# saghen/frizbee

Measured on AMD Instinct MI355X. Metric: haystacks scored/sec (whole node) + achieved HBM GB/s, 6-char needle vs 10M len-32 haystacks, higher is better.
Workload: dtype u8; 1 GPU; needle 'deadbe' (6 chars) vs 10,000,000 x 32-byte ASCII haystacks per GPU, max_typos=0, mix 5% full / 20% partial / 75% none, seed 12345 (BASELINE.json configs[1]); haystacks_per_gpu=10000000, haystack_len=32, max_typos=0, emulated_reference_backend=AVX-512 (prefilter 64 lanes, Smith-Waterman 64 x u8), ranks_seen=1, backend=none (single process), filter_survivors=499537

## Files before the change

frizbee_amd/csrc/dp_cf.h:

```cpp
#pragma once
#include "dp_body.h"

constexpr bool cf_entry_lane(int k, int s, int P) {
    if (k < 0 || k >= P) return false;
    if (s == 1) return k == P - 1;
    const int lo = P - s > 0 ? P - s : 0, hi = P - s / 2 > 0 ? P - s / 2 : 0;
    return k >= lo && k < hi;
}

struct CfRow {
    u32 orv, cmpv, cv;
    bool ci;
};
struct NeedleLongRows : NeedleLongDev {
    const u16* cf;
};
template <typename ND>
__device__ __forceinline__ CfRow cf_row_consts(const ND& nd, u32 r) {
    u32 c, f;
    if constexpr (ND::kLong) {
        const u32 cf = nd.cf[r];
        c = cf & 0xFF, f = cf >> 8;
    } else {
        c = (((const u32*)nd.c)[r >> 2] >> (8 * (r & 3))) & 0xFF, f = (((const u32*)nd.f)[r >> 2] >> (8 * (r & 3))) & 0xFF;
    }
    CfRow k;
    k.ci = c != f;
    k.orv = k.ci ? 0x00200020u : 0u;
    k.cmpv = splat16(k.ci ? (c | 0x20) : c);
    k.cv = splat16(c);
    return k;
}

template <bool UPPER>
__device__ __forceinline__ void cf_match(const CfRow& k, u32 hw, u32 bonus, u32 casev, u32& mm, u32& mb) {
    const u32 ONE = 0x00010001u;
    mm = p_subs(ONE, (hw | k.orv) ^ k.cmpv);
    mb = p_mul(mm, bonus);
    if (UPPER) {
        const u32 ex = k.ci ? p_subs(ONE, hw ^ k.cv) : mm;
        mb = p_add(mb, p_mul(ex, casev));
    }
}

template <int SWL, int REAL>
__device__ __forceinline__ void cf_scan(u32 (&b)[REAL], const u32 (&g)[REAL], u32 e, u32 lim, u32& acc0, u32& acc1) {
    constexpr int NW = SWL / 2, P = 2 * REAL;
    constexpr bool PAD = REAL < NW;
    {
        u32 cc[REAL], nb[REAL];
#pragma unroll
        for (int d = 0; d < REAL; d++) cc[d] = p_subs(b[d], g[d]);
        if (PAD && e < lim) acc1 = p_max(acc1, p_subs(cc[REAL - 1], 0xFFFFu | (((u32)P * e) << 16)));
#pragma unroll
        for (int d = 0; d < REAL; d++) nb[d] = p_max(b[d], __builtin_amdgcn_alignbit(cc[d], d ? cc[d - 1] : 0u, 16));
#pragma unroll
        for (int d = 0; d < REAL; d++) b[d] = nb[d];
    }
#pragma unroll
    for (int s = 2; s <= SWL / 2; s *= 2) {
        const int off = s / 2;
        if (PAD && (u32)s * e < lim) {
#pragma unroll
            for (int d = 0; d < REAL; d++) {
                const bool in0 = cf_entry_lane(2 * d, s, P), in1 = cf_entry_lane(2 * d + 1, s, P);
                if (in0 || in1) {
                    const u32 k0 = in0 ? (u32)(2 * d + s) * e : 0xFFFFu, k1 = in1 ? (u32)(2 * d + 1 + s) * e : 0xFFFFu;
                    const u32 v = p_subs(p_subs(b[d], g[d]), k0 | (k1 << 16));
                    if (d & 1) acc1 = p_max(acc1, v);
                    else acc0 = p_max(acc0, v);
                }
            }
        }
        if (off < REAL) {
            u32 nb[REAL];
#pragma unroll
            for (int d = 0; d < REAL; d++) nb[d] = d >= off ? p_max(b[d], p_subs(b[d - off], g[d - off])) : b[d];
#pragma unroll
            for (int d = 0; d < REAL; d++) b[d] = nb[d];
        }
    }
}

struct CfNoRowHook {
    __device__ __forceinline__ void operator()() const {}
};

template <int SWL, bool UPPER, int REAL, typename RowHook = CfNoRowHook>
__device__ __forceinline__ u32 cf_rows(const NeedleDev& nd, const u32 (&hw)[REAL], const u32 (&bonus)[REAL], const RowHook& hook = RowHook()) {
    constexpr int NW = SWL / 2;
    constexpr int P = 2 * REAL;
    constexpr bool PAD = REAL < NW;
    static_assert(REAL >= 1 && REAL <= NW, "REAL");
    static_assert(!PAD || 4 * P <= 3 * SWL, "padding entries must land inside the chunk");
    const u32 rows = (u32)nd.rows;
    const u32 e = nd.gex, x = nd.mismatch, o = nd.gopm;
    const u32 ev = splat16(e), gopmv = splat16(o), casev = splat16(nd.matching_case);
    const u32 xv = splat16(x), xqv = splat16(x - 2 * e);
    if (rows == 1) {
        const CfRow k = cf_row_consts(nd, 0);
        u32 mx = 0;
#pragma unroll
        for (int d = 0; d < REAL; d++) {
            u32 mm, mb;
            cf_match<UPPER>(k, hw[d], bonus[d], casev, mm, mb);
            mx = p_max(mx, p_subs(mb, xv));
        }
        return max(mx & 0xFFFF, mx >> 16);
    }
    u32 T[REAL], g[REAL];
    u32 acc0 = 0, acc1 = 0;
    {
        const CfRow k = cf_row_consts(nd, 0);
        u32 bias = e + (e << 17);
#pragma unroll
        for (int d = 0; d < REAL; d++, bias = fzb_sadd(bias, 2 * ev)) {
            u32 mm, mb;
            cf_match<UPPER>(k, hw[d], bonus[d], casev, mm, mb);
            T[d] = p_max(p_subs(p_add(mb, bias), xv), bias);
            g[d] = p_mul(mm, gopmv);
        }
        cf_scan<SWL, REAL>(T, g, e, (rows - 2) * o, acc0, acc1);
    }
    const u32 edc = 0xFFFFu | (((u32)(P - 2) * e + x) << 16);
    for (u32 r = 1; r + 1 < rows; r++) {
        if (r == rows / 2) hook();
        const CfRow k = cf_row_consts(nd, r);
        const u32 rb = (r + 1) * ev;
        const u32 z = ((r - 1) * e) << 16;
        if (PAD) acc0 = p_max(acc0, p_subs(T[REAL - 1], edc));
        u32 b[REAL], gn[REAL];
        u32 bias = (e << 16) + rb;
#pragma unroll
        for (int d = 0; d < REAL; d++, bias = fzb_sadd(bias, 2 * ev)) {
            const u32 sh = __builtin_amdgcn_alignbit(T[d], d ? T[d - 1] : z, 16);
            u32 mm, mb;
            cf_match<UPPER>(k, hw[d], bonus[d], casev, mm, mb);
            const u32 D = p_subs(p_add(sh, mb), xqv);
            const u32 U = p_subs(T[d], g[d]);
            b[d] = p_max3_s(D, U, bias);
            gn[d] = p_mul(mm, gopmv);
        }
        cf_scan<SWL, REAL>(b, gn, e, (rows - 2 - r) * o, acc0, acc1);
#pragma unroll
        for (int d = 0; d < REAL; d++) T[d] = b[d], g[d] = gn[d];
    }
    u32 mx;
    {
        const u32 r = rows - 1;
        const CfRow k = cf_row_consts(nd, r);
        const u32 rb = (r + 1) * ev;
        const u32 z = ((r - 1) * e) << 16;
        if (PAD) acc0 = p_max(acc0, p_subs(T[REAL - 1], edc));
        mx = p_subs(p_max(acc0, acc1), rb);
        u32 bias = (e << 16) + rb;
#pragma unroll
        for (int d = 0; d < REAL; d++, bias = fzb_sadd(bias, 2 * ev)) {
            const u32 sh = __builtin_amdgcn_alignbit(T[d], d ? T[d - 1] : z, 16);
            u32 mm, mb;
            cf_match<UPPER>(k, hw[d], bonus[d], casev, mm, mb);
            const u32 D = p_subs(p_add(sh, mb), xqv);
            const u32 U = p_subs(T[d], g[d]);
            mx = p_max(mx, p_subs(p_max(D, U), bias));
        }
    }
    return max(mx & 0xFFFF, mx >> 16);
}

template <int SWL, bool UPPER, int REAL>
__device__ __forceinline__ void cf_setup_bits(const NeedleDev& nd, bool include_prefix, const u8* cls, const u32 (&hb)[SWL / 4], u32 (&hw)[REAL], u32 (&bonus)[REAL]) {
    const u32 ONE = 0x00010001u;
    const u32 Mv = splat16(nd.match_plus_mismatch), casev = splat16(nd.matching_case), capv = splat16(nd.capitalization), delimv = splat16(nd.delimiter);
    u32 clsw_prev = 0;
#pragma unroll
    for (int d = 0; d < REAL; d++) {
        const u32 w = hb[d / 2];
        const u32 b0 = (d & 1) ? (w >> 16) & 0xFF : w & 0xFF;
        const u32 b1 = (d & 1) ? w >> 24 : (w >> 8) & 0xFF;
        hw[d] = b0 | (b1 << 16);
        const u32 clsw = (u32)cls[b0] | ((u32)cls[b1] << 16);
        const u32 sh = __builtin_amdgcn_alignbit(clsw, clsw_prev, 16);
        const u32 cap01 = (clsw >> 1) & sh & ONE;
        const u32 dl01 = (sh >> 2) & ~(clsw >> 2) & ONE;
        u32 bn = p_add(p_add(p_mul(dl01, delimv), p_mul(cap01, capv)), Mv);
        if (d == 0 && include_prefix) bn = p_add(bn, (u32)nd.prefix);
        bonus[d] = UPPER ? bn : p_add(bn, p_mul(~(clsw >> 1) & ONE, casev));
        clsw_prev = clsw;
    }
}

struct CfTables {
    u8 cls2[256];
    u16 bon[16];
};
template <bool UPPER, typename ND = NeedleDev>
__device__ __forceinline__ void cf_build_tables(const ND& nd, CfTables& t) {
    for (int b = threadIdx.x; b < 256; b += blockDim.x) {
        const bool lower = b >= 'a' && b <= 'z', upper = b >= 'A' && b <= 'Z', digit = b >= '0' && b <= '9';
        const bool delim = !(lower || upper || digit || b > 127);
        t.cls2[b] = (u8)(2 * (lower ? 1 : upper ? 2 : delim ? 3 : 0));
    }
    if (threadIdx.x < 16) {
        const u32 cp = threadIdx.x >> 2, cc = threadIdx.x & 3;
        u32 v = nd.match_plus_mismatch;
        if (cp == 3 && cc != 3) v += nd.delimiter;
        if (cc == 2 && cp == 1) v += nd.capitalization;
        if (!UPPER && cc != 2) v += nd.matching_case;
        t.bon[threadIdx.x] = (u16)v;
    }
}
template <int SWL, int REAL>
__device__ __forceinline__ void cf_setup_table(const NeedleDev& nd, bool include_prefix, const CfTables& t, const u32 (&hb)[SWL / 4], u32 (&hw)[REAL], u32 (&bonus)[REAL]) {
    u32 cprev = 0;
#pragma unroll
    for (int d = 0; d < REAL; d++) {
        hw[d] = __builtin_amdgcn_perm(0u, hb[d / 2], (d & 1) ? 0x0c030c02u : 0x0c010c00u);
        const u32 c0 = t.cls2[hw[d] & 0xFF], c1 = t.cls2[hw[d] >> 16];
// ... 72 lines not shown
```

frizbee_amd/csrc/kernels_dp.hip:

```cpp
#include "dp_cfm.h"
#include "dp_quad.h"
#include "compact1.h"
#include "seg_list.h"
#include <cstdlib>
#include <type_traits>

template <int SWL, int MODE, bool UPPER>
__global__ __launch_bounds__(128, 2) void k2b_dp(const u8* __restrict__ bytes, const EndsAny ends, u64 first, u32 index_offset,
                                              const u32* __restrict__ items, const u32* __restrict__ win, const u32* __restrict__ n_items_ptr,
                                              const NeedleDev nd, int wmode, int pad_ok, fzb_match_rec* __restrict__ out, u32 capacity, u32* __restrict__ dev_count,
                                              u32* __restrict__ overflow, u32 qcap, u32* __restrict__ counters) {
    __shared__ u8 cls[256];
    build_cls_table(cls);
    __syncthreads();
    const u32 M = __builtin_amdgcn_readfirstlane(*n_items_ptr);
    if (dev_count && blockIdx.x == 0 && threadIdx.x == 0) { dev_count[0] = M < capacity ? M : capacity; dev_count[1] = M; }
    const u64 stride = (u64)gridDim.x * blockDim.x;
    const u64 j0 = (u64)blockIdx.x * blockDim.x + threadIdx.x;
    auto load_item = [&](u64 j, u32& li, u32& ws, u32& we) {
        li = 0; ws = 0; we = 0;
        if (j < M) {
            li = items ? items[j] : (u32)j;
            if (wmode == 0) { const uint2 w = *(const uint2*)(win + 2 * j); ws = w.x; we = w.y; }
        }
// ... 42 lines not shown
            const u32 m = we - sp;
            const bool wide = m > (u32)SWL, greedy = m > FZB_MAX_HAYSTACK_LEN;
            const u32 slot_multi = wave_alloc(&counters[3], wide && !greedy);
            const u32 slot_greedy = wave_alloc(&counters[4], greedy);
            if (wide) {
                u32* qe = greedy ? overflow + 4 * (size_t)(qcap - 1 - slot_greedy) : overflow + 4 * (size_t)slot_multi;
                qe[0] = (u32)j;
                qe[1] = ws;
                qe[2] = we;
                qe[3] = li;
                break;
            }
            u32 score = 0;
            u32 hb[SWL / 4];
#pragma unroll
            for (int k = 0; k < SWL / 4; k++) hb[k] = 0;
            if (m > 0) {
                if (inreg) load_window_regs<SWL / 4>(q0_c, q1_c, sp, m, hb);
                else load_window_mem<SWL / 4>(hay + sp, m, hb);
                const bool half = pad_ok && SWL >= 16 && __all((int)(m <= (u32)SWL / 2));
                if (half) score = dp_single_chunk<SWL, MODE == 1, UPPER, (SWL >= 16 ? SWL / 4 : SWL / 2)>(nd, m, sp == 0, cls, hb);
                else score = dp_single_chunk<SWL, MODE == 1, UPPER>(nd, m, sp == 0, cls, hb);
            }
            const bool exact = exact_match<SWL / 4>(nd, include_exact, m, hb);
            if (exact) score = (score + nd.exact_bonus) & 0xFFFF;
            fzb_match_rec rec;
            rec.index = index_offset + li;
            rec.score = (u16)score;
            rec.exact = exact ? 1 : 0;
            rec.valid = 0;
            out[j] = rec;
        } while (0);
        li_c = li_n; ws_c = ws_n; we_c = we_n; s_c = s_n; L_c = L_n; q0_c = q0_n; q1_c = q1_n;
        li_n = li_m; ws_n = ws_m; we_n = we_m; s_n = s_m; L_n = L_m;
        li_m = li_f; ws_m = ws_f; we_m = we_f;
    }
}

#ifdef FZB_DP_TIMING
__device__ unsigned long long fzb_dp_timing[6 * 8192];
extern "C" int fzb_debug_dp_timing(unsigned long long* host_out) { return (int)hipMemcpyFromSymbol(host_out, HIP_SYMBOL(fzb_dp_timing), sizeof(fzb_dp_timing)); }
#define FZB_TIMING_BEGIN const unsigned long long t_rt0 = wall_clock64(), t_ck0 = clock64();
#define FZB_TIMING_END                                                                                  \
    if ((threadIdx.x & 63) == 0) {                                                                      \
        const u32 w = (blockIdx.x * blockDim.x + threadIdx.x) >> 6;                                     \
        if (w < 8192) { fzb_dp_timing[6 * w] = t_rt0; fzb_dp_timing[6 * w + 1] = wall_clock64(); fzb_dp_timing[6 * w + 2] = t_ck0; fzb_dp_timing[6 * w + 3] = clock64(); \
                        fzb_dp_timing[6 * w + 4] = __builtin_amdgcn_s_getreg(4 | (31 << 11)); fzb_dp_timing[6 * w + 5] = __builtin_amdgcn_s_getreg(20 | (31 << 11)); }  \
    }
#else
#define FZB_TIMING_BEGIN
#define FZB_TIMING_END
#endif
struct SegNone {};
template <int SWL, bool UPPER, bool SEG = false>
__global__ __launch_bounds__(128, 4) void k2b_dp_short(const u8* __restrict__ bytes, const EndsAny ends, u64 first, u32 index_offset,
                                                    const u32* __restrict__ items, const u32* __restrict__ win, const u32* __restrict__ n_items_ptr,
                                                    const NeedleDev nd, int wmode, fzb_match_rec* __restrict__ out, u32 capacity, u32* __restrict__ dev_count,
                                                    RejectOut rej, u32* __restrict__ kept_out, u32 ulen, std::conditional_t<SEG, SegList, SegNone> seg) {
    FZB_TIMING_BEGIN
    __shared__ CfTables tab;
    __shared__ u8 fl[256];
    __shared__ u32 seg_pre[SEG ? FZB_SEG_MAX : 1u];
    __shared__ u32 seg_wsum[2];
    u32 sc[16];
    if constexpr (SEG) {
        const uint4* c4 = (const uint4*)seg.counts;
#pragma unroll
        for (int k = 0; k < 4; k++) {
            const u32 i0 = 16u * threadIdx.x + 4u * k;
            const uint4 v = i0 < seg.nseg ? c4[4 * threadIdx.x + k] : make_uint4(0, 0, 0, 0);
            sc[4 * k] = v.x;
            sc[4 * k + 1] = i0 + 1 < seg.nseg ? v.y : 0u;
            sc[4 * k + 2] = i0 + 2 < seg.nseg ? v.z : 0u;
            sc[4 * k + 3] = i0 + 3 < seg.nseg ? v.w : 0u;
        }
    }
    cf_build_tables<UPPER>(nd, tab);
    if (wmode == 3) cf_build_typo_table(nd, fl);
    u32 seg_incl = 0, seg_tot = 0;
    if constexpr (SEG) {
#pragma unroll
        for (int k = 0; k < 16; k++) seg_tot += sc[k];
        seg_incl = seg_tot;
        for (int off = 1; off < 64; off <<= 1) {
            const u32 v = __shfl_up(seg_incl, off);
            if ((threadIdx.x & 63) >= (u32)off) seg_incl += v;
        }
        if ((threadIdx.x & 63) == 63) seg_wsum[threadIdx.x >> 6] = seg_incl;
    }
    __syncthreads();
    u32 M_;
    if constexpr (SEG) {
        u32 run = (threadIdx.x >= 64 ? seg_wsum[0] : 0u) + seg_incl - seg_tot;
#pragma unroll
        for (int k = 0; k < 16; k++) {
            seg_pre[16 * threadIdx.x + k] = run;
            run += sc[k];
        }
        M_ = seg_wsum[0] + seg_wsum[1];
        __syncthreads();
        if (blockIdx.x == 0 && threadIdx.x == 0) *seg.total_out = M_;
    } else {
        M_ = *n_items_ptr;
    }
    const u32 M = __builtin_amdgcn_readfirstlane(M_);
    const u32 nrej = wmode == 3 ? __builtin_amdgcn_readfirstlane(*rej.count) : 0u;
    if (blockIdx.x == 0 && threadIdx.x == 0) {
        const u32 kept = M - nrej;
        if (dev_count) { dev_count[0] = kept < capacity ? kept : capacity; dev_count[1] = kept; }
        if (kept_out) *kept_out = kept;
    }
    const u64 stride = (u64)gridDim.x * blockDim.x;
    const u64 j0 = (u64)blockIdx.x * blockDim.x + threadIdx.x;
    auto load_item = [&](u64 j, u32& li, u32& ws, u32& we) {
        li = 0; ws = 0; we = 0;
        if (j < M) {
            if constexpr (SEG) {
                const u32 sg = seg_find(seg_pre, FZB_SEG_MAX, FZB_SEG_MAX / 2, (u32)j);
                li = seg.list[(size_t)sg * seg.stride + ((u32)j - seg_pre[sg])];
            } else {
                li = items ? items[j] : (u32)j;
            }
            if (wmode == 0) { const uint2 w = *(const uint2*)(win + 2 * j); ws = w.x; we = w.y; }
        }
    };
    auto load_span = [&](u64 j, u32 li, u64& s, u32& L) {
        s = 0; L = 0;
        if (j < M) haystack_span_u(ends, ulen, first + li, s, L);
    };
    auto load_vecs = [&](u64 s, u32 L, uint4& q0, uint4& q1) {
        q0 = make_uint4(0, 0, 0, 0);
        q1 = make_uint4(0, 0, 0, 0);
        const uint4* vp = (const uint4*)(bytes + s);
        if (L > 0) q0 = vp[0];
        if (SWL > 32 && L > 16) q1 = vp[1];
    };
    u32 li_c, ws_c, we_c, L_c, li_n, ws_n, we_n, L_n, li_m, ws_m, we_m;
    u64 s_c, s_n;
    uint4 q0_c, q1_c;
    load_item(j0, li_c, ws_c, we_c);
    load_item(j0 + stride, li_n, ws_n, we_n);
    load_item(j0 + 2 * stride, li_m, ws_m, we_m);
    load_span(j0, li_c, s_c, L_c);
    load_span(j0 + stride, li_n, s_n, L_n);
    load_vecs(s_c, L_c, q0_c, q1_c);
    const u32 jw = __builtin_amdgcn_readfirstlane((u32)j0);
    const u32 n_iter = __builtin_amdgcn_readfirstlane(jw < M ? (u32)(((u64)M - jw + stride - 1) / stride) : 1u);
    struct MidItem {
        FzbProgressPrio* p;
        __device__ __forceinline__ void operator()() const { p->k2 += 1; p->apply(); }
    };
    FzbProgressPrio prio{0u, 2 * n_iter};
    for (u64 j = j0; j < M; j += stride) {
        prio.apply();
        uint4 q0_n, q1_n;
        load_vecs(s_n, L_n, q0_n, q1_n);
        u64 s_m;
        u32 L_m;
        load_span(j + 2 * stride, li_m, s_m, L_m);
        u32 li_f, ws_f, we_f;
        load_item(j + 3 * stride, li_f, ws_f, we_f);
        u64 jo = j;
        bool live = true;
        if (nrej) {
            const u32 li = li_c, tile = li / FZB_TILE;
            const u64 word = rej.bits[li >> 6];
            live = !((word >> (li & 63)) & 1);
            u32 before = rej.rej_prefix[tile] + (u32)__popcll(word & ((1ull << (li & 63)) - 1));
            for (u32 wq = tile * (FZB_TILE / 64); wq < (li >> 6); wq++) before += (u32)__popcll(rej.bits[wq]);
            jo = j - before;
        }
        if (live && jo < capacity) {
            const u32 L = L_c;
            u32 ws = ws_c, we = we_c;
            if (wmode == 2) { ws = 0; we = L; }
            else if (wmode == 1) cf_window_first_last_regs(nd, q0_c, q1_c, ws, we);
            else if (wmode == 3) cf_window_typos_regs(fl, q0_c, q1_c, L, ws, we);
            const u32 sp = ws ? ws - 1 : 0;
            const bool include_exact = sp == 0 && we == L;
            const u32 m = we - sp;
            u32 score = 0;
            u32 hb[SWL / 4];
#pragma unroll
            for (int k = 0; k < SWL / 4; k++) hb[k] = 0;
            if (m > 0) {
                load_window_regs<SWL / 4>(q0_c, q1_c, sp, m, hb);
                score = dp_single_chunk_cf_tab<SWL, UPPER, SWL / 4, MidItem>(nd, sp == 0, tab, hb, MidItem{&prio});
            }
            const bool exact = exact_match<SWL / 4>(nd, include_exact, m, hb);
            if (exact) score = (score + nd.exact_bonus) & 0xFFFF;
            fzb_match_rec rec;
            rec.index = index_offset + li_c;
            rec.score = (u16)score;
            rec.exact = exact ? 1 : 0;
            rec.valid = 0;
            out[jo] = rec;
        }
        li_c = li_n; ws_c = ws_n; we_c = we_n; s_c = s_n; L_c = L_n; q0_c = q0_n; q1_c = q1_n;
        li_n = li_m; ws_n = ws_m; we_n = we_m; s_n = s_m; L_n = L_m;
        li_m = li_f; ws_m = ws_f; we_m = we_f;
        prio.k2 = (prio.k2 | 1u) + 1;
    }
    FZB_TIMING_END
}

template <int PER>
__device__ __forceinline__ void classify_tile(u32 j0, u32 j_end, u32* s_cnt, u32* s_base, const u8* __restrict__ bytes, const EndsAny& ends, u64 first, const u32* __restrict__ items,
                                              const u32* __restrict__ win_in, const NeedleDev& nd, int wmode, u32 swl, uint4* __restrict__ meta, u32* __restrict__ lists, u32 list_stride,
                                              u32* __restrict__ overflow, u32 qcap, u32* __restrict__ counters, u32 capacity, u32 split_multi) {
    if (threadIdx.x < 9) s_cnt[threadIdx.x] = 0;
    __syncthreads();
    u32 cls[PER], rank[PER], li[PER], ws[PER], we[PER];
    const u8* src[PER];
#pragma unroll
    for (int p = 0; p < PER; p++) {
        const u32 j = j0 + p * 256 + threadIdx.x;
        cls[p] = 9; rank[p] = 0; li[p] = 0; ws[p] = 0; we[p] = 0; src[p] = bytes;
        if (j < j_end && j < capacity) {
            li[p] = items ? items[j] : j;
            u32 L = 0;
            u64 s;
            haystack_span(ends, first + li[p], s, L);
            src[p] = bytes + s;
            if (wmode == 0) { ws[p] = win_in[2 * j]; we[p] = win_in[2 * j + 1]; }
            else if (wmode == 2) { ws[p] = 0; we[p] = L; }
            else window_first_last(nd, src[p], L, ws[p], we[p]);
            const u32 sp = ws[p] ? ws[p] - 1 : 0;
            const u32 m = we[p] - sp;
            if (sp == 0 && we[p] == L) we[p] |= 0x80000000u;
            cls[p] = m <= swl / 2 ? 0u : m <= 3 * swl / 4 ? 1u : m <= swl ? 2u : m <= FZB_MAX_HAYSTACK_LEN ? 3u : 4u;
            if (split_multi && cls[p] == 3) cls[p] = 5 + ((m - 1) % swl) / (swl / 4);
            rank[p] = atomicAdd(&s_cnt[cls[p]], 1u);
        }
    }
    __syncthreads();
    if (threadIdx.x < 9 && s_cnt[threadIdx.x]) {
        const u32 c = threadIdx.x;
        s_base[c] = atomicAdd(c < 3 ? &counters[8 + c] : c == 3 ? &counters[3] : c == 4 ? &counters[4] : &counters[12 + (c - 5)], s_cnt[c]);
    }
    __syncthreads();
#pragma unroll
    for (int p = 0; p < PER; p++) {
        const u32 j = j0 + p * 256 + threadIdx.x;
        if (cls[p] < 3 || (cls[p] >= 5 && cls[p] < 9)) {
            const u32 l = cls[p] < 3 ? cls[p] : cls[p] - 2;
            lists[(size_t)l * list_stride + s_base[cls[p]] + rank[p]] = j;
            meta[j] = make_uint4(ws[p], we[p], (u32)(uintptr_t)src[p], (u32)((uintptr_t)src[p] >> 32));
        } else if (cls[p] < 5) {
            const u32 slot = s_base[cls[p]] + rank[p];
// ... 51 lines not shown
    const u32 stride = vgrid * blockDim.x;
    const u32 q0 = vblock * blockDim.x + threadIdx.x;
    auto load_meta = [&](u32 q, u32& j, u32& li, u32& sp, u32& m, u32& L, u64& s) {
        j = 0; li = 0; sp = 0; m = 0; L = 0; s = (u64)(uintptr_t)meta;
        if (q < M) {
            j = list[q];
            li = items ? items[j] : j;
            const uint4 w = meta[j];
            sp = w.x ? w.x - 1 : 0;
            m = (w.y & 0x7FFFFFFFu) - sp;
            L = w.y >> 31;
            s = (u64)w.z | ((u64)w.w << 32);
        }
    };
    auto load_bytes = [&](u64 s, u32 sp, u32 m, u32 (&hb)[NBR]) {
        const u8* th = (const u8*)(uintptr_t)s + sp;
#pragma unroll
        for (int k = 0; k < NBR; k++) {
            const u32 p = 4 * k;
            u32 v = 0;
            if (p < m) {
                v = load_u32_unaligned(th, p);
                const u32 rem = m - p;
                if (rem < 4) v &= (1u << (8 * rem)) - 1;
            }
            hb[k] = v;
        }
    };
    u32 j_c, li_c, sp_c, m_c, ex_c, j_n, li_n, sp_n, m_n, ex_n;
    u64 s_c, s_n;
    u32 hb_c[NBR];
    load_meta(q0, j_c, li_c, sp_c, m_c, ex_c, s_c);
    load_meta(q0 + stride, j_n, li_n, sp_n, m_n, ex_n, s_n);
    load_bytes(s_c, sp_c, m_c, hb_c);
    const u32 qw = __builtin_amdgcn_readfirstlane(q0);
    const u32 n_iter = __builtin_amdgcn_readfirstlane(qw < M ? (M - qw + stride - 1) / stride : 1u);
    struct MidItem {
        FzbProgressPrio* p;
        __device__ __forceinline__ void operator()() const { p->k2 += 1; p->apply(); }
    };
    FzbProgressPrio prio{0u, 2 * n_iter};
    for (u32 q = q0; q < M; q += stride) {
        prio.apply();
        u32 hb_n[NBR];
        load_bytes(s_n, sp_n, m_n, hb_n);
        u32 j_f, li_f, sp_f, m_f, ex_f;
        u64 s_f;
        load_meta(q + 2 * stride, j_f, li_f, sp_f, m_f, ex_f, s_f);
        {
            u32 hb[NB];
#pragma unroll
            for (int k = 0; k < NB; k++) hb[k] = k < NBR ? hb_c[k < NBR ? k : 0] : 0u;
            u32 score = 0;
            if (m_c > 0) score = dp_single_chunk_cf_tab<SWL, UPPER, REAL, MidItem>(nd, sp_c == 0, tab, hb, MidItem{&prio});
            const bool exact = exact_match<NB>(nd, ex_c != 0, m_c, hb);
            if (exact) score = (score + nd.exact_bonus) & 0xFFFF;
            fzb_match_rec rec;
            rec.index = index_offset + li_c;
            rec.score = (u16)score;
            rec.exact = exact ? 1 : 0;
            rec.valid = 0;
            out[j_c] = rec;
        }
        j_c = j_n; li_c = li_n; sp_c = sp_n; m_c = m_n; ex_c = ex_n; s_c = s_n;
#pragma unroll
        for (int k = 0; k < NBR; k++) hb_c[k] = hb_n[k];
        j_n = j_f; li_n = li_f; sp_n = sp_f; m_n = m_f; ex_n = ex_f; s_n = s_f;
        prio.k2 = (prio.k2 | 1u) + 1;
    }
}

template <int SWL, bool UPPER, int REAL>
__global__ __launch_bounds__(128, (REAL * 4 <= SWL ? 4 : REAL * 8 <= 3 * SWL ? 3 : 2)) void k2b_dp_class(
    u32 index_offset, const u32* __restrict__ items, const uint4* __restrict__ meta, const u32* __restrict__ list, const u32* __restrict__ n_list_ptr, const NeedleDev nd,
    fzb_match_rec* __restrict__ out) {
    __shared__ CfTables tab;
    cf_build_tables<UPPER>(nd, tab);
    __syncthreads();
    dp_class_body<SWL, UPPER, REAL>(tab, blockIdx.x, gridDim.x, index_offset, items, meta, list, n_list_ptr, nd, out);
}

void fzb_launch_compact1_classify(const CorpusDev& c, u64 first, const u64* bitmap, const u32* tile_counts, u32 n_items, u32* out_idx, u32* total_out, const NeedleDev& nd, int sw_lanes,
                                  int wmode, u32 capacity, u32* dev_count, u32* overflow, u32 qcap, u32* counters, u32* win_out, u32* lists, u32 list_stride, int grid, hipStream_t st,
                                  int split_multi) {
    FZB_LAUNCH((k_compact1_classify<3>), dim3(grid), dim3(256), 0, st, bitmap, tile_counts, n_items, out_idx, total_out, c.bytes, EndsAny{c.ends, c.ends_u64}, first, nd, wmode,
                       (u32)sw_lanes, (uint4*)win_out, lists, list_stride, overflow, qcap, counters, capacity, dev_count, (u32)split_multi);
}

void fzb_launch_dp_classes(const CorpusDev& c, u64 first, u32 index_offset, const u32* items, const u32* win_in, const u32* n_items_ptr, const NeedleDev& nd, int sw_lanes,
                           int wmode, fzb_match_rec* out, u32 capacity, u32* dev_count, u32* overflow, u32 qcap, u32* counters, u32* win_out, u32* lists, u32 list_stride,
                           int num_cus, hipStream_t st, int part, int split_multi) {
    bool upper = false;
    for (int r = 0; r < nd.rows; r++) upper = upper || (nd.c[r] >= 'A' && nd.c[r] <= 'Z');
    if (part != 2) {
#define FZB_K2W(ET) FZB_LAUNCH((k2w_classify<2>), dim3(num_cus * 8), dim3(256), 0, st, c.bytes, EndsAny{c.ends, c.ends_u64}, first, items, win_in, n_items_ptr, nd, wmode, (u32)sw_lanes, (uint4*)win_out, lists, list_stride, overflow, qcap, counters, capacity, dev_count, (u32)split_multi)
        FZB_K2W(u32);
#undef FZB_K2W
    }
    if (part == 1) return;
#define FZB_K2C(SWL, U, REAL, CLS)                                                                                                        \
    do {                                                                                                                                  \
        static int per_cu = 0;                                                                                                            \
        if (!per_cu && (hipOccupancyMaxActiveBlocksPerMultiprocessor(&per_cu, k2b_dp_class<SWL, U, REAL>, 128, 0) != hipSuccess || per_cu < 1)) per_cu = 4; \
        FZB_LAUNCH((k2b_dp_class<SWL, U, REAL>), dim3(num_cus * per_cu), dim3(128), 0, st, index_offset, items, (const uint4*)win_out, lists + (size_t)CLS * list_stride, &counters[8 + CLS], nd, out); \
    } while (0)
#define FZB_K2C_ALL(SWL, U) do { FZB_K2C(SWL, U, SWL / 4, 0); FZB_K2C(SWL, U, 3 * SWL / 8, 1); FZB_K2C(SWL, U, SWL / 2, 2); } while (0)
#define FZB_K2C_U(SWL) do { if (upper) FZB_K2C_ALL(SWL, true); else FZB_K2C_ALL(SWL, false); } while (0)
    switch (sw_lanes) {
// ... 393 lines not shown
    const u32 quad_all_below = std::min<u32>(coop_below, (u32)gm * 32u);
    const size_t dyn_lds = std::max((size_t)nd.rows * park_dw * 128 * 4, coop_below ? coop_lds : (size_t)0);
#define FZB_K2A(SWL, U) FZB_LAUNCH((k2_classes_all<SWL, U>), dim3(gm + 3 * gc), dim3(128), dyn_lds, st, index_offset, items, (const uint4*)win, lists, list_stride, counters, nd, out, capacity, scratch, (u32)gm, (u32)gc, park_dw, coop_below, quad_all_below)
#define FZB_K2A_U(SWL) do { if (upper) FZB_K2A(SWL, true); else FZB_K2A(SWL, false); } while (0)
    switch (sw_lanes) {
        case 64: FZB_K2A_U(64); break;
        case 32: FZB_K2A_U(32); break;
        case 16: FZB_K2A_U(16); break;
        default: FZB_K2A_U(8); break;
    }
}

void fzb_launch_dp_multi(const CorpusDev& c, u64 first, u32 index_offset, const u32* list, const u32* n_list_ptr, const NeedleDev& nd, int sw_lanes, int mode,
                         fzb_match_rec* out, u32 capacity, u32* scratch, int grid, hipStream_t st) {
    const int bias_ok = mode >= 1;
    if (mode == 2) {
        bool upper = false;
        for (int r = 0; r < nd.rows; r++) upper = upper || (nd.c[r] >= 'A' && nd.c[r] <= 'Z');
        const u32 park_dw = fzb_park_lds_dwords(nd, sw_lanes);
#define FZB_K2T(SWL, U, ET) FZB_LAUNCH((k2d_dp_multi_t<SWL, U>), dim3(grid), dim3(128), (size_t)nd.rows * park_dw * 128 * 4, st, c.bytes, EndsAny{c.ends, c.ends_u64}, first, index_offset, list, n_list_ptr, nd, out, capacity, scratch, park_dw)
#define FZB_K2T_ET(SWL, U) FZB_K2T(SWL, U, u32)
#define FZB_K2T_U(SWL) do { if (upper) FZB_K2T_ET(SWL, true); else FZB_K2T_ET(SWL, false); } while (0)
        switch (sw_lanes) {
            case 64: FZB_K2T_U(64); break;
            case 32: FZB_K2T_U(32); break;
            case 16: FZB_K2T_U(16); break;
            default: FZB_K2T_U(8); break;
        }
        return;
    }
#define FZB_K2D(SWL, B, ET) FZB_LAUNCH((k2d_dp_multi<SWL, B>), dim3(grid), dim3(128), 0, st, c.bytes, EndsAny{c.ends, c.ends_u64}, first, index_offset, list, n_list_ptr, nd, out, capacity, scratch)
#define FZB_K2D_ET(SWL, B) FZB_K2D(SWL, B, u32)
#define FZB_K2D_B(SWL) do { if (bias_ok) FZB_K2D_ET(SWL, true); else FZB_K2D_ET(SWL, false); } while (0)
    switch (sw_lanes) {
        case 64: FZB_K2D_B(64); break;
        case 32: FZB_K2D_B(32); break;
        case 16: FZB_K2D_B(16); break;
        default: FZB_K2D_B(8); break;
    }
}

bool fzb_dp_short_applies(const CorpusDev& c, int sw_lanes, int mode) {
    return mode == 2 && (sw_lanes == 64 || sw_lanes == 32) && c.max_len != 0 && c.max_len <= (u32)sw_lanes / 2;
}

void fzb_launch_dp(const CorpusDev& c, u64 first, u32 index_offset, const u32* items, const u32* win, const u32* n_items_ptr, const NeedleDev& nd,
                   int sw_lanes, int mode, int wmode, int pad_ok, fzb_match_rec* out, u32 capacity, u32* dev_count, u32* overflow, u32 qcap, u32* counters, int num_cus, hipStream_t st,
                   const RejectOut* rejects, const SegList* seg) {
    bool upper = false;
    for (int r = 0; r < nd.rows; r++) upper = upper || (nd.c[r] >= 'A' && nd.c[r] <= 'Z');
    if (fzb_dp_short_applies(c, sw_lanes, mode)) {
        const RejectOut rj = rejects ? *rejects : RejectOut{};
        u32* kept_out = rejects ? &counters[1] : nullptr;
#define FZB_K2S(SWL, U, SEG, SA)                                                                                                        \
    do {                                                                                                                                \
        static int per_cu = 0;                                                                                                          \
        if (!per_cu && (hipOccupancyMaxActiveBlocksPerMultiprocessor(&per_cu, k2b_dp_short<SWL, U, SEG>, 128, 0) != hipSuccess || per_cu < 1)) per_cu = 4; \
        FZB_LAUNCH((k2b_dp_short<SWL, U, SEG>), dim3(num_cus * per_cu), dim3(128), 0, st, c.bytes, EndsAny{c.ends, c.ends_u64}, first, index_offset, items, win, n_items_ptr, nd, wmode, out, capacity, dev_count, rj, kept_out, c.uniform_len, SA); \
    } while (0)
#define FZB_K2S_ET(SWL, U) do { if (seg) FZB_K2S(SWL, U, true, *seg); else FZB_K2S(SWL, U, false, SegNone{}); } while (0)
#define FZB_K2S_U(SWL) do { if (upper) FZB_K2S_ET(SWL, true); else FZB_K2S_ET(SWL, false); } while (0)
        if (sw_lanes == 64) FZB_K2S_U(64); else FZB_K2S_U(32);
        return;
    }
#define FZB_K2B(SWL, B, U, ET)                                                                                                          \
    do {                                                                                                                                \
        static int per_cu = 0;                                                                                                          \
        if (!per_cu && (hipOccupancyMaxActiveBlocksPerMultiprocessor(&per_cu, k2b_dp<SWL, B, U>, 128, 0) != hipSuccess || per_cu < 1)) per_cu = 4; \
        FZB_LAUNCH((k2b_dp<SWL, B, U>), dim3(num_cus * per_cu), dim3(128), 0, st, c.bytes, EndsAny{c.ends, c.ends_u64}, first, index_offset, items, win, n_items_ptr, nd, wmode, pad_ok, out, capacity, dev_count, overflow, qcap, counters); \
    } while (0)
#define FZB_K2B_ET(SWL, B, U) FZB_K2B(SWL, B, U, u32)
#define FZB_K2B_U(SWL, B) do { if (upper) FZB_K2B_ET(SWL, B, true); else FZB_K2B_ET(SWL, B, false); } while (0)
#define FZB_K2B_B(SWL) do { if (mode >= 1) FZB_K2B_U(SWL, 1); else FZB_K2B_U(SWL, 0); } while (0)
    switch (sw_lanes) {
        case 64: FZB_K2B_B(64); break;
        case 32: FZB_K2B_B(32); break;
        case 16: FZB_K2B_B(16); break;
        default: FZB_K2B_B(8); break;
    }
}
```

frizbee_amd/csrc/seg_list.h:

```cpp
#pragma once
#include <stdint.h>

#include "tile_compact.h"

#ifndef FZB_SEG_FN
#define FZB_SEG_FN __host__ __device__ inline
#endif

#define FZB_SEG_MAX 2048u

FZB_SEG_FN uint32_t seg_top(uint32_t nseg) {
    uint32_t top = 1;
    while (2u * top < nseg) top *= 2u;
    return top;
}
FZB_SEG_FN uint32_t seg_find(const uint32_t* pre, uint32_t nseg, uint32_t top, uint32_t j) {
    uint32_t s = 0;
#ifdef __HIP_DEVICE_COMPILE__
#pragma unroll
#endif
    for (uint32_t step = top; step; step >>= 1)
        if (s + step < nseg && pre[s + step] <= j) s += step;
    return s;
}
```

Before: 172.1 billion haystacks/s.

## Hand-schedule cf DP scan and row loops with sched barriers for ILP

Rewrites the prefix-max scan and the first, single and last DP row loops so each processes two independent dwords at a time. `sched_barrier` pins interleave the dependent packed ops so the compiler keeps them in that order. The scan entry-lane updates are software-pipelined into the shift loop, and the exact-match check is moved ahead of the DP call. The goal is to hide VALU dependency latency, at the risk of constraining the compiler scheduler and raising register pressure.

Result: no change. 173.1 billion haystacks/s (median of 6 runs) (+0.6%).

```diff
diff --git a/frizbee_amd/csrc/dp_cf.h b/frizbee_amd/csrc/dp_cf.h
--- a/frizbee_amd/csrc/dp_cf.h
+++ b/frizbee_amd/csrc/dp_cf.h
@@ -43,42 +43,127 @@
     }
 }
 
+#if defined(__HIP_DEVICE_COMPILE__)
+#define FZB_PIN() __builtin_amdgcn_sched_barrier(0x3FC)
+#else
+#define FZB_PIN() ((void)0)
+#endif
+
+constexpr int cf_entry_dwords(int s, int REAL) {
+    int n = 0;
+    for (int d = 0; d < REAL; d++) n += (cf_entry_lane(2 * d, s, 2 * REAL) || cf_entry_lane(2 * d + 1, s, 2 * REAL)) ? 1 : 0;
+    return n;
+}
+constexpr int cf_entry_first(int s, int REAL) {
+    for (int d = 0; d < REAL; d++)
+        if (cf_entry_lane(2 * d, s, 2 * REAL) || cf_entry_lane(2 * d + 1, s, 2 * REAL)) return d;
+    return 0;
+}
+constexpr u32 cf_entry_lanes(int d, int s, int P) { return (cf_entry_lane(2 * d, s, P) ? 1u : 0u) | (cf_entry_lane(2 * d + 1, s, P) ? 2u : 0u); }
+__device__ __forceinline__ u32 cf_entry_const(int d, int s, int P, u32 e) {
+    const u32 in = cf_entry_lanes(d, s, P);
+    const u32 k0 = (in & 1) ? (u32)(2 * d + s) * e : 0xFFFFu, k1 = (in & 2) ? (u32)(2 * d + 1 + s) * e : 0xFFFFu;
+    return k0 | (k1 << 16);
+}
+
 template <int SWL, int REAL>
 __device__ __forceinline__ void cf_scan(u32 (&b)[REAL], const u32 (&g)[REAL], u32 e, u32 lim, u32& acc0, u32& acc1) {
     constexpr int NW = SWL / 2, P = 2 * REAL;
     constexpr bool PAD = REAL < NW;
+    FZB_PIN();
     {
-        u32 cc[REAL], nb[REAL];
-#pragma unroll
-        for (int d = 0; d < REAL; d++) cc[d] = p_subs(b[d], g[d]);
-        if (PAD && e < lim) acc1 = p_max(acc1, p_subs(cc[REAL - 1], 0xFFFFu | (((u32)P * e) << 16)));
-#pragma unroll
-        for (int d = 0; d < REAL; d++) nb[d] = p_max(b[d], __builtin_amdgcn_alignbit(cc[d], d ? cc[d - 1] : 0u, 16));
-#pragma unroll
-        for (int d = 0; d < REAL; d++) b[d] = nb[d];
+        u32 cc[REAL];
+        const u32 k1 = (PAD && e < lim) ? 0xFFFFu | (((u32)P * e) << 16) : 0xFFFFFFFFu;
+        u32 v1 = 0;
+        cc[0] = p_subs(b[0], g[0]);
+        FZB_PIN();
+#pragma unroll
+        for (int d = 0; d < REAL; d++) {
+            if (PAD && d == REAL - 1) {
+                v1 = p_subs(cc[d], k1);
+                FZB_PIN();
+            }
+            const u32 sh = __builtin_amdgcn_alignbit(cc[d], d ? cc[d - 1] : 0u, 16);
+            FZB_PIN();
+            if (d + 1 < REAL) {
+                cc[d + 1] = p_subs(b[d + 1], g[d + 1]);
+                FZB_PIN();
+            }
+            b[d] = p_max(b[d], sh);
+            FZB_PIN();
+        }
+        if (PAD) {
+            acc1 = p_max(acc1, v1);
+            FZB_PIN();
+        }
     }
 #pragma unroll
     for (int s = 2; s <= SWL / 2; s *= 2) {
         const int off = s / 2;
-        if (PAD && (u32)s * e < lim) {
-#pragma unroll
-            for (int d = 0; d < REAL; d++) {
-                const bool in0 = cf_entry_lane(2 * d, s, P), in1 = cf_entry_lane(2 * d + 1, s, P);
-                if (in0 || in1) {
-                    const u32 k0 = in0 ? (u32)(2 * d + s) * e : 0xFFFFu, k1 = in1 ? (u32)(2 * d + 1 + s) * e : 0xFFFFu;
-                    const u32 v = p_subs(p_subs(b[d], g[d]), k0 | (k1 << 16));
-                    if (d & 1) acc1 = p_max(acc1, v);
-                    else acc0 = p_max(acc0, v);
+        const int ne = PAD ? cf_entry_dwords(s, REAL) : 0, d1 = cf_entry_first(s, REAL);
+        u32 eu = 0, ev = 0;
+        int stage = ne == 1 ? 1 : 0;
+        if (ne == 1) {
+            eu = p_subs(b[d1], g[d1]);
+            FZB_PIN();
+        }
+        const u32 ke = ne == 1 ? ((u32)s * e < lim ? cf_entry_const(d1, s, P, e) : 0xFFFFFFFFu) : 0u;
+        auto entry_next = [&]() {
+            if (stage == 1) {
+                ev = p_subs(eu, ke);
+                FZB_PIN();
+                stage = 2;
+            } else if (stage == 2) {
+                if (d1 & 1) acc1 = p_max(acc1, ev);
+                else acc0 = p_max(acc0, ev);
+                FZB_PIN();
+                stage = 0;
+            }
+        };
+        if (ne > 1 && (u32)s * e < lim) {
+#pragma unroll
+            for (int d = d1; d < d1 + ne; d += 2) {
+                const bool two = d + 1 < d1 + ne;
+                u32 ua = p_subs(b[d], g[d]), ub = 0;
+                FZB_PIN();
+                if (two) {
+                    ub = p_subs(b[d + 1], g[d + 1]);
+                    FZB_PIN();
                 }
+                ua = p_subs(ua, cf_entry_const(d, s, P, e));
+                FZB_PIN();
+                if (two) {
+                    ub = p_subs(ub, cf_entry_const(d + 1, s, P, e));
+                    FZB_PIN();
+                }
+                if (d & 1) acc1 = p_max(acc1, ua);
+                else acc0 = p_max(acc0, ua);
+                FZB_PIN();
+                if (two) {
+                    if (d & 1) acc0 = p_max(acc0, ub);
+                    else acc1 = p_max(acc1, ub);
+                    FZB_PIN();
+                }
             }
         }
         if (off < REAL) {
-            u32 nb[REAL];
-#pragma unroll
-            for (int d = 0; d < REAL; d++) nb[d] = d >= off ? p_max(b[d], p_subs(b[d - off], g[d - off])) : b[d];
-#pragma unroll
-            for (int d = 0; d < REAL; d++) b[d] = nb[d];
-        }
+            u32 t = p_subs(b[REAL - 1 - off], g[REAL - 1 - off]);
+            FZB_PIN();
+#pragma unroll
+            for (int d = REAL - 1; d >= off; d--) {
+                u32 tn = 0;
+                if (d - 1 >= off) {
+                    tn = p_subs(b[d - 1 - off], g[d - 1 - off]);
+                    FZB_PIN();
+                }
+                entry_next();
+                b[d] = p_max(b[d], t);
+                FZB_PIN();
+                t = tn;
+            }
+        }
+        entry_next();
+        entry_next();
     }
 }
 
@@ -99,13 +184,24 @@
     const u32 xv = splat16(x), xqv = splat16(x - 2 * e);
     if (rows == 1) {
         const CfRow k = cf_row_consts(nd, 0);
-        u32 mx = 0;
-#pragma unroll
-        for (int d = 0; d < REAL; d++) {
-            u32 mm, mb;
-            cf_match<UPPER>(k, hw[d], bonus[d], casev, mm, mb);
-            mx = p_max(mx, p_subs(mb, xv));
-        }
+        u32 mx = 0, mx1 = 0;
+#pragma unroll
+        for (int d = 0; d < REAL; d += 2) {
+            const int db = d + 1 < REAL ? d + 1 : d;
+            u32 mma, mba, mmb, mbb;
+            cf_match<UPPER>(k, hw[d], bonus[d], casev, mma, mba);
+            cf_match<UPPER>(k, hw[db], bonus[db], casev, mmb, mbb);
+            FZB_PIN();
+            const u32 sa = p_subs(mba, xv);
+            FZB_PIN();
+            const u32 sb = p_subs(mbb, xv);
+            FZB_PIN();
+            mx = p_max(mx, sa);
+            FZB_PIN();
+            mx1 = p_max(mx1, sb);
+            FZB_PIN();
+        }
+        mx = p_max(mx, mx1);
         return max(mx & 0xFFFF, mx >> 16);
     }
     u32 T[REAL], g[REAL];
@@ -114,11 +210,27 @@
         const CfRow k = cf_row_consts(nd, 0);
         u32 bias = e + (e << 17);
 #pragma unroll
-        for (int d = 0; d < REAL; d++, bias = fzb_sadd(bias, 2 * ev)) {
-            u32 mm, mb;
-            cf_match<UPPER>(k, hw[d], bonus[d], casev, mm, mb);
-            T[d] = p_max(p_subs(p_add(mb, bias), xv), bias);
-            g[d] = p_mul(mm, gopmv);
+        for (int d = 0; d < REAL; d += 2) {
+            const int db = d + 1 < REAL ? d + 1 : d;
+            const u32 bias_b = db != d ? fzb_sadd(bias, 2 * ev) : bias;
+            u32 mma, mba, mmb, mbb;
+            cf_match<UPPER>(k, hw[d], bonus[d], casev, mma, mba);
+            cf_match<UPPER>(k, hw[db], bonus[db], casev, mmb, mbb);
+            const u32 da = p_add(mba, bias), dbv = p_add(mbb, bias_b);
+            FZB_PIN();
+            const u32 sa = p_subs(da, xv);
+            FZB_PIN();
+            const u32 sb = p_subs(dbv, xv);
+            FZB_PIN();
+            T[d] = p_max(sa, bias);
+            FZB_PIN();
+            T[db] = p_max(sb, bias_b);
+            FZB_PIN();
+            g[d] = p_mul(mma, gopmv);
+            FZB_PIN();
+            g[db] = p_mul(mmb, gopmv);
+            FZB_PIN();
+            bias = fzb_sadd(bias_b, 2 * ev);
         }
         cf_scan<SWL, REAL>(T, g, e, (rows - 2) * o, acc0, acc1);
     }
@@ -151,18 +263,53 @@
         const CfRow k = cf_row_consts(nd, r);
         const u32 rb = (r + 1) * ev;
         const u32 z = ((r - 1) * e) << 16;
-        if (PAD) acc0 = p_max(acc0, p_subs(T[REAL - 1], edc));
-        mx = p_subs(p_max(acc0, acc1), rb);
+        const u32 ea = PAD ? p_subs(T[REAL - 1], edc) : 0u;
+        u32 mx1 = 0;
+        mx = 0;
         u32 bias = (e << 16) + rb;
 #pragma unroll
-        for (int d = 0; d < REAL; d++, bias = fzb_sadd(bias, 2 * ev)) {
-            const u32 sh = __builtin_amdgcn_alignbit(T[d], d ? T[d - 1] : z, 16);
-            u32 mm, mb;
-            cf_match<UPPER>(k, hw[d], bonus[d], casev, mm, mb);
-            const u32 D = p_subs(p_add(sh, mb), xqv);
-            const u32 U = p_subs(T[d], g[d]);
-            mx = p_max(mx, p_subs(p_max(D, U), bias));
-        }
+        for (int d = 0; d < REAL; d += 2) {
+            const int db = d + 1 < REAL ? d + 1 : d;
+            const u32 bias_b = db != d ? fzb_sadd(bias, 2 * ev) : bias;
+            const u32 sha = __builtin_amdgcn_alignbit(T[d], d ? T[d - 1] : z, 16), shb = __builtin_amdgcn_alignbit(T[db], db ? T[db - 1] : z, 16);
+            u32 mma, mba, mmb, mbb;
+            cf_match<UPPER>(k, hw[d], bonus[d], casev, mma, mba);
+            cf_match<UPPER>(k, hw[db], bonus[db], casev, mmb, mbb);
+            const u32 da = p_add(sha, mba), dbv = p_add(shb, mbb);
+            const u32 Ua = p_subs(T[d], g[d]), Ub = p_subs(T[db], g[db]);
+            FZB_PIN();
+            const u32 Da = p_subs(da, xqv);
+            FZB_PIN();
+            const u32 bias_next = fzb_sadd(bias_b, 2 * ev);
+            const u32 Db = p_subs(dbv, xqv);
+            FZB_PIN();
+            if (d == 0 && PAD) {
+                acc0 = p_max(acc0, ea);
+                FZB_PIN();
+            }
+            const u32 ca = p_max(Da, Ua);
+            FZB_PIN();
+            if (d == 0) {
+                mx = p_max(acc0, acc1);
+                FZB_PIN();
+            }
+            const u32 cb = p_max(Db, Ub);
+            FZB_PIN();
+            if (d == 0) {
+                mx = p_subs(mx, rb);
+                FZB_PIN();
+            }
+            const u32 pa = p_subs(ca, bias);
+            FZB_PIN();
+            const u32 pb = p_subs(cb, bias_b);
+            FZB_PIN();
+            mx = p_max(mx, pa);
+            FZB_PIN();
+            mx1 = p_max(mx1, pb);
+            FZB_PIN();
+            bias = bias_next;
+        }
+        mx = p_max(mx, mx1);
     }
     return max(mx & 0xFFFF, mx >> 16);
 }
diff --git a/frizbee_amd/csrc/kernels_dp.hip b/frizbee_amd/csrc/kernels_dp.hip
--- a/frizbee_amd/csrc/kernels_dp.hip
+++ b/frizbee_amd/csrc/kernels_dp.hip
@@ -249,11 +249,9 @@
             u32 hb[SWL / 4];
 #pragma unroll
             for (int k = 0; k < SWL / 4; k++) hb[k] = 0;
-            if (m > 0) {
-                load_window_regs<SWL / 4>(q0_c, q1_c, sp, m, hb);
-                score = dp_single_chunk_cf_tab<SWL, UPPER, SWL / 4, MidItem>(nd, sp == 0, tab, hb, MidItem{&prio});
-            }
+            if (m > 0) load_window_regs<SWL / 4>(q0_c, q1_c, sp, m, hb);
             const bool exact = exact_match<SWL / 4>(nd, include_exact, m, hb);
+            if (m > 0) score = dp_single_chunk_cf_tab<SWL, UPPER, SWL / 4, MidItem>(nd, sp == 0, tab, hb, MidItem{&prio});
             if (exact) score = (score + nd.exact_bonus) & 0xFFFF;
             fzb_match_rec rec;
             rec.index = index_offset + li_c;
@@ -418,8 +416,8 @@
 #pragma unroll
             for (int k = 0; k < NB; k++) hb[k] = k < NBR ? hb_c[k < NBR ? k : 0] : 0u;
             u32 score = 0;
+            const bool exact = exact_match<NB>(nd, ex_c != 0, m_c, hb);
             if (m_c > 0) score = dp_single_chunk_cf_tab<SWL, UPPER, REAL, MidItem>(nd, sp_c == 0, tab, hb, MidItem{&prio});
-            const bool exact = exact_match<NB>(nd, ex_c != 0, m_c, hb);
             if (exact) score = (score + nd.exact_bonus) & 0xFFFF;
             fzb_match_rec rec;
             rec.index = index_offset + li_c;
```

## Map segment items directly to owning blocks in short DP kernel, pool the remainder

Applied to the files above, without the earlier changes.

The segmented-list path of the short DP kernel gets its own device function. Block b now takes up to 128 items of segment b directly, one per thread, and starts loading that haystack before the prefix scan finishes. Only the overflow items go through a global pool, which needs a binary search over a second prefix array. This is meant to remove the per-item binary search over segment prefixes and to overlap the first global loads with the block-wide scan, at the cost of more shared memory (a second 2048-entry prefix array) and more involved indexing. The per-item DP scoring code is also factored into a shared helper.

After: 172.1 billion haystacks/s before, 181.1 billion haystacks/s after, median of 6. +5.2%, better.

```diff
diff --git a/frizbee_amd/csrc/kernels_dp.hip b/frizbee_amd/csrc/kernels_dp.hip
--- a/frizbee_amd/csrc/kernels_dp.hip
+++ b/frizbee_amd/csrc/kernels_dp.hip
@@ -118,58 +118,181 @@
 #define FZB_TIMING_END
 #endif
 struct SegNone {};
+template <int SWL, bool UPPER, class Mid>
+__device__ __forceinline__ void dp_short_item(const NeedleDev& nd, const CfTables& tab, const uint4& q0, const uint4& q1, u32 L, u32 ws, u32 we, u32 index,
+                                              fzb_match_rec* __restrict__ dst, Mid mid) {
+    const u32 sp = ws ? ws - 1 : 0;
+    const bool include_exact = sp == 0 && we == L;
+    const u32 m = we - sp;
+    u32 score = 0;
+    u32 hb[SWL / 4];
+#pragma unroll
+    for (int k = 0; k < SWL / 4; k++) hb[k] = 0;
+    if (m > 0) {
+        load_window_regs<SWL / 4>(q0, q1, sp, m, hb);
+        score = dp_single_chunk_cf_tab<SWL, UPPER, SWL / 4, Mid>(nd, sp == 0, tab, hb, mid);
+    }
+    const bool exact = exact_match<SWL / 4>(nd, include_exact, m, hb);
+    if (exact) score = (score + nd.exact_bonus) & 0xFFFF;
+    fzb_match_rec rec;
+    rec.index = index;
+    rec.score = (u16)score;
+    rec.exact = exact ? 1 : 0;
+    rec.valid = 0;
+    *dst = rec;
+}
+
+template <int SWL, bool UPPER>
+__device__ __forceinline__ void dp_short_seg(const u8* __restrict__ bytes, const EndsAny& ends, u64 first, u32 index_offset, const NeedleDev& nd,
+                                             fzb_match_rec* __restrict__ out, u32 capacity, u32* __restrict__ dev_count, u32* __restrict__ kept_out, u32 ulen,
+                                             const SegList& seg) {
+    __shared__ CfTables tab;
+    __shared__ u32 seg_pre[FZB_SEG_MAX];
+    __shared__ u32 seg_rpre[FZB_SEG_MAX];
+    __shared__ u32 seg_wsum[4];
+    constexpr u32 NONE = 0xFFFFFFFFu;
+    const u32 b = blockIdx.x, G = gridDim.x, t = threadIdx.x;
+    const u32 wg_size = blockDim.x;
+    __builtin_assume(wg_size == FZB_SEG_DIRECT);
+    auto load_span = [&](u32 jo, u32 li, u64& s, u32& L) {
+        s = 0; L = 0;
+        if (jo != NONE) haystack_span_u(ends, ulen, first + li, s, L);
+    };
+    auto load_vecs = [&](u64 s, u32 L, uint4& q0, uint4& q1) {
+        q0 = make_uint4(0, 0, 0, 0);
+        q1 = make_uint4(0, 0, 0, 0);
+        const uint4* vp = (const uint4*)(bytes + s);
+        if (L > 0) q0 = vp[0];
+        if (SWL > 32 && L > 16) q1 = vp[1];
+    };
+    const bool own = b < seg.nseg;
+    u32 lane_zero = t;
+    asm volatile("" : "+v"(lane_zero));
+    const u32 cb_any = seg.counts[(own ? b : 0u) + (lane_zero >> 31)];
+    u32 sc[16];
+    const uint4* c4 = (const uint4*)seg.counts;
+#pragma unroll
+    for (int k = 0; k < 4; k++) {
+        const u32 i0 = 16u * t + 4u * k;
+        const uint4 v = c4[4 * t + k];
+        sc[4 * k] = i0 < seg.nseg ? v.x : 0u;
+        sc[4 * k + 1] = i0 + 1 < seg.nseg ? v.y : 0u;
+        sc[4 * k + 2] = i0 + 2 < seg.nseg ? v.z : 0u;
+        sc[4 * k + 3] = i0 + 3 < seg.nseg ? v.w : 0u;
+    }
+    cf_build_tables<UPPER>(nd, tab);
+    const bool has_c = own && t < seg_direct(cb_any, b, G);
+    u32 li_c = 0;
+    if (has_c) li_c = seg.list[(size_t)b * seg.stride + t];
+    u32 sr[16], tot = 0, rtot = 0;
+#pragma unroll
+    for (int k = 0; k < 16; k++) {
+        sr[k] = seg_rest(sc[k], 16u * t + k, G);
+        tot += sc[k];
+        rtot += sr[k];
+    }
+    asm volatile("" : "+v"(tot), "+v"(rtot));
+    u32 jo_c = has_c ? 0u : NONE;
+    u64 s_c;
+    u32 L_c;
+    uint4 q0_c, q1_c;
+    load_span(jo_c, li_c, s_c, L_c);
+    load_vecs(s_c, L_c, q0_c, q1_c);
+    u32 incl = tot, rincl = rtot;
+    for (int off = 1; off < 64; off <<= 1) {
+        const u32 v = __shfl_up(incl, off), rv = __shfl_up(rincl, off);
+        if ((t & 63) >= (u32)off) { incl += v; rincl += rv; }
+    }
+    if ((t & 63) == 63) { seg_wsum[t >> 6] = incl; seg_wsum[2 + (t >> 6)] = rincl; }
+    __syncthreads();
+    const u32 M = __builtin_amdgcn_readfirstlane(seg_wsum[0] + seg_wsum[1]);
+    const u32 R = __builtin_amdgcn_readfirstlane(seg_wsum[2] + seg_wsum[3]);
+    {
+        u32 run = (t >= 64 ? seg_wsum[0] : 0u) + incl - tot, rrun = (t >= 64 ? seg_wsum[2] : 0u) + rincl - rtot;
+        if (R) {
+#pragma unroll
+            for (int k = 0; k < 16; k++) {
+                seg_pre[16 * t + k] = run;
+                seg_rpre[16 * t + k] = rrun;
+                run += sc[k];
+                rrun += sr[k];
+            }
+        } else {
+#pragma unroll
+            for (int k = 0; k < 16; k++) {
+                if (16 * t + k == b) seg_pre[b] = run;
+                run += sc[k];
+            }
+        }
+    }
+    __syncthreads();
+    if (b == 0 && t == 0) {
+        *seg.total_out = M;
+        if (dev_count) { dev_count[0] = M < capacity ? M : capacity; dev_count[1] = M; }
+        if (kept_out) *kept_out = M;
+    }
+    if (has_c) jo_c = seg_pre[own ? b : 0u] + t;
+    const u32 stride = G * FZB_SEG_DIRECT, j0 = b * FZB_SEG_DIRECT + t;
+    auto load_pool = [&](u64 jp, u32& li, u32& jo) {
+        li = 0; jo = NONE;
+        if (jp < R) {
+            const SegItem it = seg_pool_item(seg_pre, seg_rpre, FZB_SEG_MAX, FZB_SEG_MAX / 2, G, (u32)jp);
+            li = seg.list[(size_t)it.seg * seg.stride + it.slot];
+            jo = it.pos;
+        }
+    };
+    u32 li_n, jo_n, L_n, li_m, jo_m;
+    u64 s_n;
+    load_pool(j0, li_n, jo_n);
+    load_pool((u64)j0 + stride, li_m, jo_m);
+    load_span(jo_n, li_n, s_n, L_n);
+    const u32 jw = __builtin_amdgcn_readfirstlane(j0);
+    const u32 n_pool = jw < R ? (R - jw - 1u) / stride + 1u : 0u;
+    const u32 n_iter = (n_pool || __any((int)has_c)) ? 1u + n_pool : 0u;
+    struct MidItem {
+        FzbProgressPrio* p;
+        __device__ __forceinline__ void operator()() const { p->k2 += 1; p->apply(); }
+    };
+    FzbProgressPrio prio{0u, 2 * n_iter};
+    u64 jp_f = (u64)j0 + 2 * (u64)stride;
+    for (u32 k = 0; k < n_iter; k++, jp_f += stride) {
+        prio.apply();
+        uint4 q0_n, q1_n;
+        load_vecs(s_n, L_n, q0_n, q1_n);
+        u64 s_m;
+        u32 L_m;
+        load_span(jo_m, li_m, s_m, L_m);
+        u32 li_f, jo_f;
+        load_pool(jp_f, li_f, jo_f);
+        if (jo_c < capacity) {
+            u32 ws, we;
+            cf_window_first_last_regs(nd, q0_c, q1_c, ws, we);
+            dp_short_item<SWL, UPPER>(nd, tab, q0_c, q1_c, L_c, ws, we, index_offset + li_c, &out[jo_c], MidItem{&prio});
+        }
+        li_c = li_n; jo_c = jo_n; s_c = s_n; L_c = L_n; q0_c = q0_n; q1_c = q1_n;
+        li_n = li_m; jo_n = jo_m; s_n = s_m; L_n = L_m;
+        li_m = li_f; jo_m = jo_f;
+        prio.k2 = (prio.k2 | 1u) + 1;
+    }
+}
+
 template <int SWL, bool UPPER, bool SEG = false>
 __global__ __launch_bounds__(128, 4) void k2b_dp_short(const u8* __restrict__ bytes, const EndsAny ends, u64 first, u32 index_offset,
                                                     const u32* __restrict__ items, const u32* __restrict__ win, const u32* __restrict__ n_items_ptr,
                                                     const NeedleDev nd, int wmode, fzb_match_rec* __restrict__ out, u32 capacity, u32* __restrict__ dev_count,
                                                     RejectOut rej, u32* __restrict__ kept_out, u32 ulen, std::conditional_t<SEG, SegList, SegNone> seg) {
     FZB_TIMING_BEGIN
+    if constexpr (SEG) {
+        dp_short_seg<SWL, UPPER>(bytes, ends, first, index_offset, nd, out, capacity, dev_count, kept_out, ulen, seg);
+        FZB_TIMING_END
+        return;
+    }
     __shared__ CfTables tab;
     __shared__ u8 fl[256];
-    __shared__ u32 seg_pre[SEG ? FZB_SEG_MAX : 1u];
-    __shared__ u32 seg_wsum[2];
-    u32 sc[16];
-    if constexpr (SEG) {
-        const uint4* c4 = (const uint4*)seg.counts;
-#pragma unroll
-        for (int k = 0; k < 4; k++) {
-            const u32 i0 = 16u * threadIdx.x + 4u * k;
-            const uint4 v = i0 < seg.nseg ? c4[4 * threadIdx.x + k] : make_uint4(0, 0, 0, 0);
-            sc[4 * k] = v.x;
-            sc[4 * k + 1] = i0 + 1 < seg.nseg ? v.y : 0u;
-            sc[4 * k + 2] = i0 + 2 < seg.nseg ? v.z : 0u;
-            sc[4 * k + 3] = i0 + 3 < seg.nseg ? v.w : 0u;
-        }
-    }
     cf_build_tables<UPPER>(nd, tab);
     if (wmode == 3) cf_build_typo_table(nd, fl);
-    u32 seg_incl = 0, seg_tot = 0;
-    if constexpr (SEG) {
-#pragma unroll
-        for (int k = 0; k < 16; k++) seg_tot += sc[k];
-        seg_incl = seg_tot;
-        for (int off = 1; off < 64; off <<= 1) {
-            const u32 v = __shfl_up(seg_incl, off);
-            if ((threadIdx.x & 63) >= (u32)off) seg_incl += v;
-        }
-        if ((threadIdx.x & 63) == 63) seg_wsum[threadIdx.x >> 6] = seg_incl;
-    }
-    __syncthreads();
-    u32 M_;
-    if constexpr (SEG) {
-        u32 run = (threadIdx.x >= 64 ? seg_wsum[0] : 0u) + seg_incl - seg_tot;
-#pragma unroll
-        for (int k = 0; k < 16; k++) {
-            seg_pre[16 * threadIdx.x + k] = run;
-            run += sc[k];
-        }
-        M_ = seg_wsum[0] + seg_wsum[1];
-        __syncthreads();
-        if (blockIdx.x == 0 && threadIdx.x == 0) *seg.total_out = M_;
-    } else {
-        M_ = *n_items_ptr;
-    }
-    const u32 M = __builtin_amdgcn_readfirstlane(M_);
+    __syncthreads();
+    const u32 M = __builtin_amdgcn_readfirstlane(*n_items_ptr);
     const u32 nrej = wmode == 3 ? __builtin_amdgcn_readfirstlane(*rej.count) : 0u;
     if (blockIdx.x == 0 && threadIdx.x == 0) {
         const u32 kept = M - nrej;
@@ -181,12 +304,7 @@
     auto load_item = [&](u64 j, u32& li, u32& ws, u32& we) {
         li = 0; ws = 0; we = 0;
         if (j < M) {
-            if constexpr (SEG) {
-                const u32 sg = seg_find(seg_pre, FZB_SEG_MAX, FZB_SEG_MAX / 2, (u32)j);
-                li = seg.list[(size_t)sg * seg.stride + ((u32)j - seg_pre[sg])];
-            } else {
-                li = items ? items[j] : (u32)j;
-            }
+            li = items ? items[j] : (u32)j;
             if (wmode == 0) { const uint2 w = *(const uint2*)(win + 2 * j); ws = w.x; we = w.y; }
         }
     };
@@ -242,25 +360,7 @@
             if (wmode == 2) { ws = 0; we = L; }
             else if (wmode == 1) cf_window_first_last_regs(nd, q0_c, q1_c, ws, we);
             else if (wmode == 3) cf_window_typos_regs(fl, q0_c, q1_c, L, ws, we);
-            const u32 sp = ws ? ws - 1 : 0;
-            const bool include_exact = sp == 0 && we == L;
-            const u32 m = we - sp;
-            u32 score = 0;
-            u32 hb[SWL / 4];
-#pragma unroll
-            for (int k = 0; k < SWL / 4; k++) hb[k] = 0;
-            if (m > 0) {
-                load_window_regs<SWL / 4>(q0_c, q1_c, sp, m, hb);
-                score = dp_single_chunk_cf_tab<SWL, UPPER, SWL / 4, MidItem>(nd, sp == 0, tab, hb, MidItem{&prio});
-            }
-            const bool exact = exact_match<SWL / 4>(nd, include_exact, m, hb);
-            if (exact) score = (score + nd.exact_bonus) & 0xFFFF;
-            fzb_match_rec rec;
-            rec.index = index_offset + li_c;
-            rec.score = (u16)score;
-            rec.exact = exact ? 1 : 0;
-            rec.valid = 0;
-            out[jo] = rec;
+            dp_short_item<SWL, UPPER>(nd, tab, q0_c, q1_c, L, ws, we, index_offset + li_c, &out[jo], MidItem{&prio});
         }
         li_c = li_n; ws_c = ws_n; we_c = we_n; s_c = s_n; L_c = L_n; q0_c = q0_n; q1_c = q1_n;
         li_n = li_m; ws_n = ws_m; we_n = we_m; s_n = s_m; L_n = L_m;
@@ -919,7 +1019,8 @@
     if (fzb_dp_short_applies(c, sw_lanes, mode)) {
         const RejectOut rj = rejects ? *rejects : RejectOut{};
         u32* kept_out = rejects ? &counters[1] : nullptr;
-#define FZB_K2S(SWL, U, SEG, SA)                                                                                                        \
+        static_assert(FZB_SEG_DIRECT == 128, "dp_short_seg takes one direct item per thread and tells the compiler its workgroup has FZB_SEG_DIRECT threads: the launch below must have as many");
+#define FZB_K2S(SWL, U, SEG, SA)                                                                                                     \
     do {                                                                                                                                \
         static int per_cu = 0;                                                                                                          \
         if (!per_cu && (hipOccupancyMaxActiveBlocksPerMultiprocessor(&per_cu, k2b_dp_short<SWL, U, SEG>, 128, 0) != hipSuccess || per_cu < 1)) per_cu = 4; \
diff --git a/frizbee_amd/csrc/seg_list.h b/frizbee_amd/csrc/seg_list.h
--- a/frizbee_amd/csrc/seg_list.h
+++ b/frizbee_amd/csrc/seg_list.h
@@ -23,3 +23,20 @@
         if (s + step < nseg && pre[s + step] <= j) s += step;
     return s;
 }
+
+#define FZB_SEG_DIRECT 128u
+
+FZB_SEG_FN uint32_t seg_direct(uint32_t c, uint32_t s, uint32_t G) { return s < G ? (c < FZB_SEG_DIRECT ? c : FZB_SEG_DIRECT) : 0u; }
+FZB_SEG_FN uint32_t seg_rest(uint32_t c, uint32_t s, uint32_t G) { return c - seg_direct(c, s, G); }
+FZB_SEG_FN uint32_t seg_pool_first(uint32_t s, uint32_t G) { return s < G ? FZB_SEG_DIRECT : 0u; }
+
+struct SegItem {
+    uint32_t seg, slot, pos;
+};
+FZB_SEG_FN SegItem seg_pool_item(const uint32_t* pre, const uint32_t* rpre, uint32_t nseg, uint32_t top, uint32_t G, uint32_t jp) {
+    SegItem it;
+    it.seg = seg_find(rpre, nseg, top, jp);
+    it.slot = seg_pool_first(it.seg, G) + (jp - rpre[it.seg]);
+    it.pos = pre[it.seg] + it.slot;
+    return it;
+}
```
